# MaxLayar/Ray-Tracing-Extended

Measured on AMD Instinct MI355X. Metric: Mrays/s, higher is better.
Workload: dtype f32; 1 GPU; configs[2]: Chess pieces x17 (100,440 triangles, BVH4), 1920x1080, 64 rays/pixel/frame (1024 spp = 16 frames), 8 bounces, PCG, FLAT_CHUNKS semantics; decomposition=single GPU, rays_per_frame=243378252, triangles=100440, chunks=7448, spheres=0

## Files before the change

### ray-tracing-extended_amd/csrc/rt_api.hip

```cpp
#include <hip/hip_runtime.h>

#include <algorithm>
#include <chrono>
#include <cfloat>
#include <cmath>
#include <condition_variable>
#include <deque>
#include <mutex>
#include <cstdarg>
#include <cstdio>
#include <cstring>
#include <ctime>
#include <string>
#include <thread>
#include <vector>

#include "rt_kernels.hpp"
#include "rt_stream.hpp"
namespace rtk {
const void* stream_kernel(bool counting, bool philox, bool compact, bool triangles);
const void* cam_stream_kernel(bool philox, bool compact, bool triangles);
}
#include "rt_geom.hpp"
#include "rt_bvh_gpu.hpp"
// ... 38 lines not shown
    int row0 = 0, nrows = -1;
    int band_first = 0, band_stride = 0;

    std::vector<rt_sphere>   h_spheres;
    std::vector<rt_triangle> h_tris;
    std::vector<rt_meshinfo> h_mesh;
    bool scene_dirty = true;
    size_t n_tris = 0, n_chunks = 0, n_spheres = 0;
    float sphere_mag = 0.f;
    bool geom_local = false, xf_dirty = false;
    uint64_t frames_traced = 0, frames_at_world_build = ~0ull;
    std::vector<rt_triangle>       h_local_tris;
    std::vector<rt_local_chunk>    h_lchunks;
    std::vector<rt_mesh_transform> h_xf;
    std::vector<float>             mesh_radius;
    int n_meshes = 0;
    DevBuf<float> d_local_tris;
    DevBuf<uint32_t> d_tri_mesh, d_tri_chunk, d_tri_rank, d_order;
    DevBuf<rtg::MeshXf> d_xf;
    hipEvent_t evg0 = nullptr, evg1 = nullptr;
    hipEvent_t ev_switch = nullptr;

    DevBuf<float4> d_sph_geom, d_sph_mat, d_nodes, d_nodes_h, d_tri_geo, d_tri_nrm, d_chunk_mat, d_chunk_box;
    DevBuf<float>  d_raw_tris;
    DevBuf<uint32_t> d_raw_range;
    DevBuf<float4> d_frame, d_accum;
    DevBuf<uint32_t> d_display;
    DevBuf<float4> d_batch;
    DevBuf<uint32_t> d_tile_order, d_tile_cost, d_tile_hist;
    bool lpt_active = true;
    bool tile_order_valid = false, tile_order_stale = false; int tile_order_n = 0;
    size_t target_pixels = 0;
    int target_w = 0, target_h = 0, target_row0 = 0, target_rows = 0, target_row_stride = 8;
    unsigned int* d_tile_counter = nullptr;
    unsigned long long* d_counters = nullptr;

    rtbvh::Bvh bvh;
    size_t n_nodes = 0;
    rtgb::Workspace bvh_ws;
    float area_at_build = 0.f;
    float area_after_refit = 0.f;
    int opt_device_bvh = -1;
    int opt_bvh_radius = -16;
    int opt_peer_copies = 0;
    int opt_bvh_treelet_ratio = 8, opt_bvh_treelet_isolate = 1, opt_bvh_treelet_first = 1;
    int opt_bvh_treelets = 6;
    int opt_bvh_top = 0;
    int opt_rebuild_percent = 200;
    int n_cu = 0;
    int opt_kernel = -1;
    int auto_choice = -1; double auto_ms[2] = { -1.0, -1.0 };
    unsigned variants_launched = 0;
    int opt_shade_threshold = 48;
    int opt_tile_sync = 1;
    int opt_fetch_guide = 4;
    int opt_fetch_guide_philox = 1;
    int opt_tiles_per_fetch = 16;
    int opt_compact_nodes = 1;
    int opt_stream_tile = 4;
    int opt_node_min = 10;
    int opt_blocks_per_cu = 0;
    int opt_full_sort = 0;
    int opt_tile_lpt = 1;
    int opt_frame_batch = 0;
    int opt_tile_w_log2 = 3;
    int opt_bvh_reinsert = 0;
    int opt_bvh_bins = 32, opt_bvh_cost_exp = 100;
    int opt_max_leaf = 2;
    int opt_bvh_collapse = 0;
    int opt_bvh_node_cost = 130;
    int opt_stream_stack = 0;
    int opt_lds_stack = 0;
    DevBuf<uint32_t> d_gstack;
    DevBuf<uint4> d_primary; DevBuf<float4> d_focus; DevBuf<unsigned int> d_primary_counts;
    std::string primary_key;
    unsigned long long scene_version = 0;
    int opt_primary_lists = 1;
    DevBuf<float> d_park;
    std::vector<rtk::CamRecord> h_cams; DevBuf<rtk::CamRecord> d_cams;
    DevBuf<float4> d_q_rays, d_q_hits; DevBuf<uint8_t> d_q_occ;
    DevBuf<unsigned int> d_q_bound;
    DevBuf<float4> d_aov[RT_AOV_COUNT];
    size_t aov_pixels = 0;
    int aov_w = 0, aov_h = 0, aov_row0 = 0, aov_rows = 0, aov_row_stride = 8;
    rt_aov_info aov{};
    rt_stats stats{};

    std::thread q_thread; bool q_started = false;
    std::mutex q_mu; std::condition_variable q_cv, q_idle;
    struct QItem { int frame; rt_params p; };
    std::deque<QItem> q_frames; bool q_busy = false, q_stop = false;
    rt_params q_tail{};
    int q_rc = 0; std::string q_err;
    int opt_queue_depth = 64;
    int opt_queue_linger_us = 200;
};

namespace {

int fail(rt_ctx* ctx, int code, const char* fmt, ...)
{
    char buf[512];
    va_list ap; va_start(ap, fmt); vsnprintf(buf, sizeof buf, fmt, ap); va_end(ap);
    if (ctx) ctx->err = buf; else g_create_error = buf;
    return code;
}
// ... 477 lines not shown
        F.tile_w_log2 = c->opt_tile_w_log2;
        const int tw = 1 << F.tile_w_log2, th = 64 >> F.tile_w_log2;
        F.tiles_x = (c->target_w + tw - 1) / tw; F.tiles_y = (c->target_rows + th - 1) / th;
    }
    const bool philox = P.philox = c->params.rngMode == RT_RNG_PHILOX && c->params.numRaysPerPixel >= 1;
    if (philox && var == Variant::Flat) return fail(c, -2, "the flat validation kernel implements the PCG stream only");
    if (philox) kernel = 1;
    if (philox && (c->target_w > 65535 || c->target_rows > 65535)) return fail(c, -7, "the Philox mode addresses at most 65535 x 65535 pixels per context");
    if (philox && (c->params.numRaysPerPixel > 65000 || c->params.maxBounceCount > 32000))
        return fail(c, -7, "the Philox mode takes at most 65000 rays per pixel per frame and 32000 bounces (sample and bounce share one signed 32-bit register)");
    const bool stream = P.stream = kernel == 1 && var != Variant::Flat && c->params.numRaysPerPixel >= 1
                                   && c->target_w <= 65535 && c->target_rows <= 65535
                                   && c->params.numRaysPerPixel <= 65000 && c->params.maxBounceCount <= 32000;
    const bool tile_kernel = P.tile_kernel = !stream && var != Variant::Flat;
    F.stack_cap = tile_kernel ? tile_stack_cap(c)
                              : std::max(1, c->bvh.maxStack) + (stream ? 3 : 0);
    const bool seven_waves = stream && !philox && var == Variant::Fast && c->opt_compact_nodes != 0 && c->n_nodes > 0;
    const int stream_stack = c->opt_stream_stack > 0 ? c->opt_stream_stack : (seven_waves ? (RT_STREAM_WAVES >= 7 ? 21 : 24) : 30);
    const bool stream_spill = stream && F.stack_cap > stream_stack;
    if (stream_spill) F.stack_cap = stream_stack;
    F.full_sort = c->opt_full_sort;
    bool fixed_origin = camera_origin_is_fixed(c->params);
    if (cams) for (int f = 0; f < n_frames; ++f) fixed_origin = fixed_origin && camera_origin_is_fixed(cams[f]);
    F.fixed_origin = fixed_origin ? 1 : 0;
    F.out_frame = c->d_frame.p; F.accum = c->d_accum.p;
    F.tile_counter = c->d_tile_counter; F.counters = c->d_counters;

    const size_t lds = P.lds = var == Variant::Flat ? 0
                                       : (size_t)F.stack_cap * 64 * sizeof(uint32_t) * rtk::kWavesPerBlock
                                         + (stream ? (size_t)rtk::kGroupMax * sizeof(uint2) * rtk::kWavesPerBlock : 0);
    if (lds > 160 * 1024) return fail(c, -7, "BVH needs a %d-entry traversal stack: exceeds the 160 KiB LDS", F.stack_cap);
    const bool counting = var == Variant::Counting;
    const bool compact = c->opt_compact_nodes != 0;
    P.cam_table = cams != nullptr;
    const void* fn = P.fn = var == Variant::Flat ? (const void*)rtk::k_trace<false, true>
                   : stream ? (cams ? rtk::cam_stream_kernel(philox, compact, c->n_nodes > 0)
                                    : rtk::stream_kernel(counting, philox, compact, c->n_nodes > 0))
                   : c->n_nodes == 0
                            ? dispatch3(counting, false, false, [](auto C, auto, auto) { return (const void*)rtk::k_trace<decltype(C)::value, false, false, 6>; })
                            : dispatch3(counting, false, compact, [](auto C, auto, auto H) { return (const void*)rtk::k_trace<decltype(C)::value, false, decltype(H)::value>; });
    if (lds > 64 * 1024) RT_HIP(c, hipFuncSetAttribute(fn, hipFuncAttributeMaxDynamicSharedMemorySize, (int)lds));
    int per_cu = 0;
    RT_HIP(c, hipOccupancyMaxActiveBlocksPerMultiprocessor(&per_cu, fn, rtk::kBlock, lds));
    if (per_cu < 1) return fail(c, -7, "kernel does not fit a CU (LDS %zu B)", lds);
    P.ntiles = F.tiles_x * F.tiles_y;
    P.sample_lanes_log2 = !philox ? 0 : c->params.numRaysPerPixel >= 16 ? 4 : c->params.numRaysPerPixel >= 4 ? 2 : 0;
    const bool stream_sync = P.stream_sync = stream && (c->opt_tile_sync || philox);
    if (cams && !stream_sync) return fail(c, -7, "per-frame cameras: no k_cam_stream launch for this target");
    const size_t frames_in_queue = ((stream_sync && c->opt_frame_batch != 1) ? (size_t)std::max(1, std::min(n_frames, 64)) : 1) << P.sample_lanes_log2;
    const int want = (int)std::min<size_t>(((size_t)P.ntiles * frames_in_queue + rtk::kWavesPerBlock - 1) / rtk::kWavesPerBlock, (size_t)1 << 20);
    if (c->opt_blocks_per_cu > 0) per_cu = std::min(per_cu, c->opt_blocks_per_cu);
    const int grid = P.grid = std::max(1, std::min(want, per_cu * c->n_cu));
    A.shade_threshold = std::max(1, std::min(64, c->opt_shade_threshold));
    A.total_pixels = (unsigned int)P.ntiles * 64u;
    A.tile_sync = stream_sync ? 1 : 0;
    A.sample_lanes_log2 = P.sample_lanes_log2;
    A.tiles_per_fetch = std::max(1, std::min(rtk::kGroupMax, c->opt_tiles_per_fetch));
    A.guide_div = 1;
    A.node_min = std::max(1, std::min(64, c->opt_node_min));
    const unsigned int gstack_stride = (unsigned int)grid * rtk::kBlock;
    if (philox) {
        RT_HIP(c, c->d_park.ensure((size_t)grid * rtk::kWavesPerBlock * (size_t)A.tiles_per_fetch * 192));
        F.park = c->d_park.p;
    }
    if (stream_spill) {
        RT_HIP(c, c->d_gstack.ensure((size_t)(c->bvh.maxStack + 3 - F.stack_cap) * gstack_stride));
        F.gstack = c->d_gstack.p; F.gstack_stride = gstack_stride;
    }
    if (tile_kernel && c->bvh.maxStack > F.stack_cap) {
        RT_HIP(c, c->d_gstack.ensure((size_t)(c->bvh.maxStack - F.stack_cap) * gstack_stride));
        F.gstack = c->d_gstack.p; F.gstack_stride = gstack_stride;
    }
    if ((tile_kernel || stream_sync) && n_frames > 1 && c->opt_frame_batch != 1) {
        const size_t budget = (size_t)4 << 30;
        const size_t per_frame = c->target_pixels * sizeof(float4);
        int batch = (int)std::min<size_t>((size_t)n_frames, std::max<size_t>(1, budget / per_frame));
        if (c->opt_frame_batch > 1) batch = std::min(batch, c->opt_frame_batch);
        P.batch = batch = std::min(batch, 256);
        if (batch > 1) RT_HIP(c, c->d_batch.ensure((size_t)batch * c->target_pixels));
    }
    return 0;
}

int plan_tile_order(rt_ctx* c, LaunchPlan& P)
{
    const int ntiles = P.ntiles;
    const bool lpt = (P.tile_kernel || P.stream_sync) && c->opt_tile_lpt && ntiles > 1;
    c->lpt_active = lpt;
    if (!lpt) return 0;
    if (c->tile_order_n != ntiles) { c->tile_order_valid = false; c->tile_order_n = ntiles; }
    RT_HIP(c, c->d_tile_cost.ensure(ntiles)); RT_HIP(c, c->d_tile_order.ensure(ntiles));
    if (!c->tile_order_valid || c->tile_order_stale) {
        P.record_costs = true;
        RT_HIP(c, hipMemsetAsync(c->d_tile_cost.p, 0, (size_t)ntiles * sizeof(uint32_t), c->stream));
    }
    P.F.tile_order = c->tile_order_valid ? c->d_tile_order.p : nullptr;
    P.F.tile_cost = P.record_costs ? c->d_tile_cost.p : nullptr;
    return 0;
}

int ensure_primary_lists(rt_ctx* c, LaunchPlan& P)
{
    const bool eligible = P.stream && !P.cam_table && c->opt_primary_lists && c->n_nodes > 0 && P.F.fixed_origin && c->target_pixels > 0
                          && c->bvh.maxStack <= 160;
    if (!eligible) return 0;
    std::string key((const char*)&c->params, sizeof c->params);
// ... 606 lines not shown
        }
    }
    for (int t = 0; t < n_tris; ++t) if (!seen[t]) return fail(c, -5, "triangle %d belongs to no chunk", t);
    for (float& r : radius) r *= 1.7320508f;
    c->h_local_tris.assign(tris, tris + n_tris); c->h_lchunks.assign(chunks, chunks + n_chunks);
    c->mesh_radius = radius; c->n_meshes = n_meshes;
    c->geom_local = true; c->scene_dirty = true;
    return 0;
}

int rt_set_mesh_transforms(rt_ctx* c, const rt_mesh_transform* xf, int n_meshes)
{
    if (!c) return -1;
    RT_SETTLE(c);
    if (n_meshes < 0 || (n_meshes > 0 && !xf)) return fail(c, -2, "bad transform upload");
    if (c->geom_local && n_meshes != c->n_meshes) return fail(c, -2, "%d transforms for %d meshes", n_meshes, c->n_meshes);
    c->h_xf.assign(xf, xf + n_meshes);
    c->xf_dirty = true;
    return 0;
}

int rt_read_world_geometry(rt_ctx* c, rt_triangle* tris_out, int n_tris, rt_meshinfo* mi_out, int n_chunks)
{
    if (!c) return -1;
    RT_SETTLE(c);
    if (!c->geom_local) return fail(c, -2, "no local meshes uploaded");
    if (!c->have_params) return fail(c, -2, "rt_set_params has not been called");
    if (n_tris != (int)c->h_local_tris.size() || n_chunks != (int)c->h_lchunks.size()) return fail(c, -2, "size mismatch");
    RT_HIP(c, hipSetDevice(c->device));
    { int r = prepare_scene(c); if (r) return r; }
    if (n_tris) RT_HIP(c, hipMemcpy(tris_out, c->d_raw_tris.p, (size_t)n_tris * sizeof(rt_triangle), hipMemcpyDeviceToHost));
    std::vector<float4> box(2 * (size_t)n_chunks);
    if (n_chunks) RT_HIP(c, hipMemcpy(box.data(), c->d_chunk_box.p, box.size() * sizeof(float4), hipMemcpyDeviceToHost));
    for (int m = 0; m < n_chunks; ++m) {
        const rt_local_chunk& ch = c->h_lchunks[m];
        rt_meshinfo& mi = mi_out[m];
        mi.firstTriangleIndex = ch.firstTriangleIndex; mi.numTriangles = ch.numTriangles; mi.material = ch.material;
        mi.boundsMin[0] = box[2 * m].x; mi.boundsMin[1] = box[2 * m].y; mi.boundsMin[2] = box[2 * m].z;
        mi.boundsMax[0] = box[2 * m + 1].x; mi.boundsMax[1] = box[2 * m + 1].y; mi.boundsMax[2] = box[2 * m + 1].z;
    }
    return 0;
}

int rt_set_option(rt_ctx* c, const char* name, int value)
{
    if (!c) return -1;
    RT_SETTLE(c);
    if (!name) return fail(c, -2, "null option name");
    if (!std::strcmp(name, "kernel")) {
        if (value < -1 || value > 1) return fail(c, -2, "kernel must be -1 (auto), 0 (k_trace) or 1 (k_stream)");
        c->opt_kernel = value;
    }
    else if (!std::strcmp(name, "shade_threshold")) { if (value < 1 || value > 64) return fail(c, -2, "shade_threshold must be in [1,64]"); c->opt_shade_threshold = value; }
    else if (!std::strcmp(name, "stream_stack")) { if (value != 0 && (value < 4 || value > 128)) return fail(c, -2, "stream_stack must be 0 (automatic) or in [4,128]"); c->opt_stream_stack = value; }
    else if (!std::strcmp(name, "lds_stack")) { if (value < 0 || value > 64) return fail(c, -2, "lds_stack must be in [0,64]"); c->opt_lds_stack = value; }
    else if (!std::strcmp(name, "bvh_bins")) { if (value < 2 || value > 128) return fail(c, -2, "bvh_bins must be in [2,128]"); if (value != c->opt_bvh_bins) c->scene_dirty = true; c->opt_bvh_bins = value; }
    else if (!std::strcmp(name, "bvh_reinsert")) { if (value < 0 || value > 16) return fail(c, -2, "bvh_reinsert must be in [0,16]"); if (value != c->opt_bvh_reinsert) c->scene_dirty = true; c->opt_bvh_reinsert = value; }
    else if (!std::strcmp(name, "bvh_cost_exp")) { if (value < 10 || value > 300) return fail(c, -2, "bvh_cost_exp must be in [10,300] (percent)"); if (value != c->opt_bvh_cost_exp) c->scene_dirty = true; c->opt_bvh_cost_exp = value; }
    else if (!std::strcmp(name, "max_leaf")) { if (value < 1 || value > rtbvh::kMaxLeaf) return fail(c, -2, "max_leaf must be in [1,4]"); if (value != c->opt_max_leaf) c->scene_dirty = true; c->opt_max_leaf = value; }
    else if (!std::strcmp(name, "bvh_collapse")) { if (value < 0 || value > 2) return fail(c, -2, "bvh_collapse must be 0 (greedy), 1 (cost-driven, leaves formed by the collapse) or 2 (cost-driven over the split search's leaves)"); if (value != c->opt_bvh_collapse) c->scene_dirty = true; c->opt_bvh_collapse = value; }
    else if (!std::strcmp(name, "bvh_node_cost")) { if (value < 1 || value > 10000) return fail(c, -2, "bvh_node_cost must be in [1,10000] (percent of a triangle test)"); if (value != c->opt_bvh_node_cost) c->scene_dirty = true; c->opt_bvh_node_cost = value; }
    else if (!std::strcmp(name, "tile_w_log2")) { if (value < 0 || value > 6) return fail(c, -2, "tile_w_log2 must be in [0,6]"); c->opt_tile_w_log2 = value; }
    else if (!std::strcmp(name, "tile_lpt")) { c->opt_tile_lpt = value ? 1 : 0; c->tile_order_valid = false; }
    else if (!std::strcmp(name, "frame_batch")) { if (value < 0 || value > 1024) return fail(c, -2, "frame_batch must be in [0,1024]"); c->opt_frame_batch = value; }
    else if (!std::strcmp(name, "fetch_guide")) { if (value < 1 || value > 64) return fail(c, -2, "fetch_guide must be in [1,64]"); c->opt_fetch_guide = value; }
    else if (!std::strcmp(name, "fetch_guide_philox")) { if (value < 1 || value > 64) return fail(c, -2, "fetch_guide_philox must be in [1,64]"); c->opt_fetch_guide_philox = value; }
    else if (!std::strcmp(name, "tiles_per_fetch")) { if (value < 1 || value > 64) return fail(c, -2, "tiles_per_fetch must be in [1,64]"); c->opt_tiles_per_fetch = value; }
    else if (!std::strcmp(name, "node_min")) { if (value < 1 || value > 64) return fail(c, -2, "node_min must be in [1,64]"); c->opt_node_min = value; }
    else if (!std::strcmp(name, "tile_sync")) c->opt_tile_sync = value ? 1 : 0;
    else if (!std::strcmp(name, "compact_nodes")) c->opt_compact_nodes = value ? 1 : 0;
    else if (!std::strcmp(name, "device_bvh")) { if (value < -1 || value > 1) return fail(c, -2, "device_bvh must be -1 (automatic), 0 or 1"); if (value != c->opt_device_bvh) c->scene_dirty = true; c->opt_device_bvh = value; }
    else if (!std::strcmp(name, "bvh_radius")) { if (value == 0 || value < -rtgb::kMaxRadius || value > rtgb::kMaxRadius) return fail(c, -2, "bvh_radius must be in [1,64] (negative: the same radius in every round)"); if (value != c->opt_bvh_radius) c->scene_dirty = true; c->opt_bvh_radius = value; }
    else if (!std::strcmp(name, "peer_copies")) { if (value != 0 && value != 1) return fail(c, -2, "peer_copies must be 0 or 1"); c->opt_peer_copies = value; }
    else if (!std::strcmp(name, "bvh_treelet_ratio")) { if (value < 2 || value > 64) return fail(c, -2, "bvh_treelet_ratio must be in [2,64]"); if (value != c->opt_bvh_treelet_ratio) c->scene_dirty = true; c->opt_bvh_treelet_ratio = value; }
    else if (!std::strcmp(name, "bvh_treelet_isolate")) { if (value < 0 || value > 1) return fail(c, -2, "bvh_treelet_isolate must be 0 or 1"); if (value != c->opt_bvh_treelet_isolate) c->scene_dirty = true; c->opt_bvh_treelet_isolate = value; }
    else if (!std::strcmp(name, "bvh_treelet_first")) { if (value < 1 || value > 4096) return fail(c, -2, "bvh_treelet_first must be in [1,4096]"); if (value != c->opt_bvh_treelet_first) c->scene_dirty = true; c->opt_bvh_treelet_first = value; }
    else if (!std::strcmp(name, "bvh_treelets")) { if (value < 0 || value > 16) return fail(c, -2, "bvh_treelets must be in [0,16] (passes)"); if (value != c->opt_bvh_treelets) c->scene_dirty = true; c->opt_bvh_treelets = value; }
    else if (!std::strcmp(name, "bvh_top")) { if (value < 0 || value > (1 << 20)) return fail(c, -2, "bvh_top must be in [0,1048576] (0 = the device's clustering builds the whole tree)"); if (value != c->opt_bvh_top) c->scene_dirty = true; c->opt_bvh_top = value; }
    else if (!std::strcmp(name, "rebuild_percent")) { if (value < 0 || value > 100000) return fail(c, -2, "rebuild_percent must be in [0,100000] (0 = never rebuild)"); c->opt_rebuild_percent = value; }
    else if (!std::strcmp(name, "stream_tile")) { if (value != 0 && value != 2 && value != 4) return fail(c, -2, "stream_tile must be 0 (8x8 pixels x 1 frame), 2 (4x4 x 4 frames) or 4 (2x2 x 16 frames)"); c->opt_stream_tile = value; }
    else if (!std::strcmp(name, "full_sort")) c->opt_full_sort = value ? 1 : 0;
    else if (!std::strcmp(name, "primary_lists")) { if (value != 0 && value != 1) return fail(c, -2, "primary_lists must be 0 or 1"); c->opt_primary_lists = value; }
    else if (!std::strcmp(name, "queue_depth")) { if (value < 1 || value > 256) return fail(c, -2, "queue_depth must be in [1,256]"); c->opt_queue_depth = value; }
    else if (!std::strcmp(name, "queue_linger_us")) { if (value < 0 || value > 1000000) return fail(c, -2, "queue_linger_us must be in [0,1000000]"); c->opt_queue_linger_us = value; }
    else if (!std::strcmp(name, "blocks_per_cu")) { if (value < 0) return fail(c, -2, "blocks_per_cu must be >= 0"); c->opt_blocks_per_cu = value; }
    else return fail(c, -2, "unknown option '%s'", name);
    return 0;
}

int rt_set_rows(rt_ctx* c, int row0, int nrows)
{
    if (!c) return -1;
    RT_SETTLE(c);
    if (row0 < 0 || nrows < 0) return fail(c, -2, "bad row strip (%d,%d)", row0, nrows);
    c->row0 = row0; c->nrows = nrows; c->band_stride = 0;
    return 0;
}

int rt_set_bands(rt_ctx* c, int first_band, int band_stride)
{
    if (!c) return -1;
    RT_SETTLE(c);
    if (first_band < 0 || band_stride < 1 || first_band >= band_stride) return fail(c, -2, "bad band pattern (%d,%d)", first_band, band_stride);
    c->band_first = first_band; c->band_stride = band_stride;
    return 0;
}
// ... 581 lines not shown
```

### ray-tracing-extended_amd/csrc/rt_stream.hpp

```cpp
#pragma once
#include "rt_kernels.hpp"

namespace rtk {

struct StreamArgs {
    int shade_threshold;
    unsigned int total_pixels;
    int node_min;
    int tiles_per_fetch;
    int guide_div;
    int tile_sync;
    int n16, n4, n1;
    int sample_lanes_log2;
};

enum : uint32_t { kModeTrav = 0, kModeShade = 1, kModeDead = 2, kModeWait = 3, kModeTravStrict = 0xFFFFFFFFu };
__device__ __forceinline__ bool is_trav(uint32_t mode) { return (int)mode <= 0; }
constexpr uint32_t kNoPixel = 0xFFFFFFFFu;

struct StreamKernArgs { DeviceScene S; FrameArgs F; StreamArgs A; };
static_assert(alignof(StreamArgs) <= 8, "kernarg layout = struct layout");
static_assert(offsetof(StreamKernArgs, F) == ((sizeof(DeviceScene) + 7) & ~size_t(7))
              && offsetof(StreamKernArgs, A) == ((offsetof(StreamKernArgs, F) + sizeof(FrameArgs) + 7) & ~size_t(7)), "kernarg layout = struct layout");

struct CamRecord {
    float4 view;
    float4 m0, m1, m2;
    float4 pos;
};
struct StreamCamKernArgs { DeviceScene S; FrameArgs F; StreamArgs A; const CamRecord* cams; };
static_assert(offsetof(StreamCamKernArgs, A) == offsetof(StreamKernArgs, A)
              && offsetof(StreamCamKernArgs, cams) == ((offsetof(StreamCamKernArgs, A) + sizeof(StreamArgs) + 7) & ~size_t(7)), "kernarg layout = struct layout");

#ifndef RT_STREAM_WAVES
#define RT_STREAM_WAVES 7
#endif
#ifndef RT_STREAM_WAVES_PHILOX
#define RT_STREAM_WAVES_PHILOX 5
#endif
constexpr int stream_waves(bool count, bool philox, bool h, bool tri) { return count ? 3 : !tri ? 6 : philox ? RT_STREAM_WAVES_PHILOX : !h ? 5 : RT_STREAM_WAVES; }


template <bool COUNT, bool PHILOX = false, bool H = false, bool TRI = true>
__global__ __launch_bounds__(kBlock) __attribute__((amdgpu_waves_per_eu(stream_waves(COUNT, PHILOX, H, TRI), stream_waves(COUNT, PHILOX, H, TRI)))) void k_stream(DeviceScene S, FrameArgs F, StreamArgs A)
{
    constexpr bool CAMS = false;
#include "rt_stream_body.hpp"
}

template <bool PHILOX, bool H, bool TRI>
__global__ __launch_bounds__(kBlock) __attribute__((amdgpu_waves_per_eu(stream_waves(false, PHILOX, H, TRI), stream_waves(false, PHILOX, H, TRI)))) void k_cam_stream(DeviceScene S, FrameArgs F, StreamArgs A, const CamRecord* cams)
{
    constexpr bool COUNT = false, CAMS = true;
    (void)cams;
#include "rt_stream_body.hpp"
}

}
```

### ray-tracing-extended_amd/csrc/rt_stream_body.hpp

```cpp
    extern __shared__ uint32_t lds_stack[];
    RT_MARK("begin prologue");
    const int lane = threadIdx.x & 63, wave = threadIdx.x >> 6;
    uint32_t* stk = lds_stack + (size_t)wave * F.stack_cap * 64 + lane;
    const int cap = F.stack_cap;
    uint32_t* const gstk = F.gstack ? F.gstack + (blockIdx.x * kBlock + threadIdx.x) : nullptr;
    using lds_u32 = __attribute__((address_space(3))) uint32_t;
    const uint32_t stk0 = (uint32_t)(uintptr_t)(lds_u32*)stk;
    uint32_t top = stk0;
    auto slot = [](uint32_t a) -> lds_u32& { return *reinterpret_cast<lds_u32*>((uintptr_t)a); };
    const uint32_t capb = (uint32_t)cap << 8;
    uint32_t ub = 0u;
    auto pop = [&]() -> uint32_t {
        top -= 256u;
        if (gstk == nullptr || ub <= capb) return slot(top);
        RT_RARE_PATH();
        const uint32_t depth = top - stk0;
        uint32_t v = slot(stk0 + min(depth, capb - 256u));
        asm volatile("" : "+v"(v));
        if (depth >= capb) { RT_RARE_PATH(); v = gstk[(size_t)((depth - capb) >> 8) * F.gstack_stride]; }
        return v;
    };
    typedef uint32_t u32x2 __attribute__((ext_vector_type(2)));
    using lds_u2 = __attribute__((address_space(3))) u32x2;
    lds_u2* const item_tab = reinterpret_cast<lds_u2*>((uintptr_t)__builtin_amdgcn_readfirstlane(
// ... 10 lines not shown
    uint32_t rng = 0u;
    int sample = 0;
    v3 total = rtm::mk(0.f, 0.f, 0.f), light = total, rayColour = total, o = total, d = total;
    RaySlabT<H> slab = make_slab<H>(rtm::mk(0.f, 0.f, 0.f), rtm::mk(1.f, 1.f, 1.f));
    uint32_t cur = kNone;
    Hit best; best.t = INF; best.id = kNone; best.u = 0.f; best.v = 0.f;
    bool live = false;
    unsigned long long wave_t0 = 0;
    unsigned int group_base = 0, group_len = 0;
    unsigned int next_unit = 0;
    unsigned int kidx = 0;

    auto decode = [](const FrameArgs& F, const StreamArgs& A, unsigned int item, unsigned int& tile, unsigned int& sub, unsigned int& frame0) -> int {
        const unsigned int ntiles_ = (unsigned)(F.tiles_x * F.tiles_y);
        if constexpr (PHILOX) {
            const int sgl = A.sample_lanes_log2;
            const unsigned int per_frame = ntiles_ << sgl;
            const unsigned int g = item / per_frame, r = item - g * per_frame;
            tile = r >> sgl; sub = r & ((1u << sgl) - 1u); frame0 = g;
            return sgl;
        }
        const unsigned int items1_ = (unsigned)A.n1 * ntiles_, items4_ = (unsigned)A.n4 * (ntiles_ << 2);
        int fgl = 0; unsigned int fbase = (unsigned)A.n16 * 16u + (unsigned)A.n4 * 4u;
        if (item >= items1_) { item -= items1_; fgl = 2; fbase = (unsigned)A.n16 * 16u; if (item >= items4_) { item -= items4_; fgl = 4; fbase = 0u; } }
        const unsigned int per_group = ntiles_ << fgl;
        const unsigned int g = item / per_group, r = item - g * per_group;
        tile = r >> fgl; sub = r & ((1u << fgl) - 1u); frame0 = fbase + (g << fgl);
        return fgl;
    };
    auto pixel_index = [&](const FrameArgs& F) -> uint32_t {
        const int ly = (int)(pxy >> 16);
        return (uint32_t)(F.row0 + (ly >> 3) * F.row_stride + (ly & 7)) * (uint32_t)F.p.width + (pxy & 0xFFFFu);
    };
    auto start_pixel = [&](const FrameArgs& F, const StreamArgs& A, unsigned int id) -> bool {
        const rt_params& p = F.p;
        const uint32_t W = (uint32_t)p.width;
        const unsigned int nframes_ = (unsigned)(A.n16 * 16 + A.n4 * 4 + A.n1);
        const u32x2 e = item_tab[id >> 6];
        const unsigned int pos = id & 63u;
        const int fgl = (int)(e.y >> 28);
        const unsigned int frame0 = e.y & 0x0FFFFFFFu;
        const int pxl = 6 - fgl, swl = pxl >> 1;
        const unsigned int pix = pos & ((1u << pxl) - 1u);
        const unsigned int fi = PHILOX ? frame0 : frame0 + (pos >> pxl);
        const int x = (int)((e.x & 0xFFFFu) + (pix & ((1u << swl) - 1u)));
        const int yy = (int)((e.x >> 16) + (pix >> swl));
        if (!(x < p.width && yy < F.nrows && fi < nframes_)) return false;
        pxy = (uint32_t)x | ((uint32_t)yy << 16); kidx = id | (fi << 16);
        const uint32_t pixelIndex = (uint32_t)(F.row0 + (yy >> 3) * F.row_stride + (yy & 7)) * W + (uint32_t)x;
        if constexpr (PHILOX) sample = (int)(pos >> pxl);
        else { rng = pixelIndex + (uint32_t)(F.frame + (int)fi) * 719393u; sample = 0; }
        total = rtm::mk(0.f, 0.f, 0.f);
        live = false;
        return true;
    };
    auto take_units = [&](const FrameArgs& F, const StreamArgs& A, bool want) -> bool {
        bool got = false;
        const unsigned int total_units = group_len << 6;
        for (;;) {
            const unsigned long long need = ballot_(want);
            if (need == 0ull || next_unit >= total_units) break;
            if (want) {
                const unsigned int id = next_unit + __builtin_amdgcn_mbcnt_hi((uint32_t)(need >> 32), __builtin_amdgcn_mbcnt_lo((uint32_t)need, 0u));
                if (id < total_units && start_pixel(F, A, id)) { want = false; got = true; }
            }
            next_unit = __builtin_amdgcn_readfirstlane(min(total_units, next_unit + (unsigned int)__popcll(need)));
        }
        return got;
    };

    RT_MARK("end prologue");
    for (;;) {
        const int nTrav = __popcll(ballot_(is_trav(mode))), nShade = __popcll(ballot_(mode == kModeShade));
        if (nTrav + nShade == 0) {
            if (!A.tile_sync) break;
            RT_REGION_BEGIN(fetch);
            const StreamKernArgs& KA = fresh_kernargs<StreamKernArgs>();
            const FrameArgs& F = KA.F; const StreamArgs& A = KA.A;
            const unsigned int ntiles_ = (unsigned)(F.tiles_x * F.tiles_y);
            const unsigned int nitems_ = PHILOX ? (unsigned)A.n1 * (ntiles_ << A.sample_lanes_log2)
                                                : (unsigned)A.n1 * ntiles_ + (unsigned)A.n4 * (ntiles_ << 2) + (unsigned)A.n16 * (ntiles_ << 4);
            if constexpr (PHILOX) {
                const int pxl = 6 - A.sample_lanes_log2, swl = pxl >> 1;
                const uint32_t W = (uint32_t)F.p.width;
                const float nf = (float)F.p.numRaysPerPixel;
                asm volatile("s_waitcnt vmcnt(0)" ::: "memory");
                for (unsigned int k = 0; k < group_len; ++k) {
                    const u32x2 e = item_tab[k];
                    const unsigned int fi = e.y & 0x0FFFFFFFu;
                    const unsigned int pix = (unsigned)lane & ((1u << pxl) - 1u);
                    const int x = (int)((e.x & 0xFFFFu) + (pix & ((1u << swl) - 1u)));
                    const int yy = (int)((e.x >> 16) + (pix >> swl));
                    const bool present = x < F.p.width && yy < F.nrows;
                    float tx = 0.f, ty = 0.f, tz = 0.f;
                    if (present) {
                        const float* q = park_slot(F, A, k) + lane;
                        tx = __hip_atomic_load(q, __ATOMIC_RELAXED, __HIP_MEMORY_SCOPE_AGENT);
                        ty = __hip_atomic_load(q + 64, __ATOMIC_RELAXED, __HIP_MEMORY_SCOPE_AGENT);
                        tz = __hip_atomic_load(q + 128, __ATOMIC_RELAXED, __HIP_MEMORY_SCOPE_AGENT);
                    }
                    for (int off = 1 << pxl; off < 64; off <<= 1) {
                        tx = tx + __shfl_xor(tx, off, 64); ty = ty + __shfl_xor(ty, off, 64); tz = tz + __shfl_xor(tz, off, 64);
                    }
                    if (present && ((unsigned)lane >> pxl) == 0u) {
                        const float cx = tx / nf, cy = ty / nf, cz = tz / nf;
                        const size_t pi = (size_t)yy * W + (uint32_t)x;
                        F.out_frame[(size_t)fi * F.frame_stride + pi] = make_float4(cx, cy, cz, 1.0f);
                        if (F.frames_in_launch <= 1) {
                            const float weight = 1.0f / (float)(F.frame + 1);
                            const float omw = 1.0f - weight;
                            const float4 prev = F.accum[pi];
                            float4 acc;
                            acc.x = rtm::saturate(prev.x * omw + cx * weight);
                            acc.y = rtm::saturate(prev.y * omw + cy * weight);
                            acc.z = rtm::saturate(prev.z * omw + cz * weight);
                            acc.w = rtm::saturate(prev.w * omw + 1.0f * weight);
                            F.accum[pi] = acc;
                        }
                    }
                }
            }
            uint32_t slot = (uint32_t)lane;
            asm volatile("" : "+v"(slot));
            if (F.tile_cost && group_len != 0 && slot < group_len) {
                const uint32_t share = (uint32_t)(((__builtin_readcyclecounter() - wave_t0) >> 6) / group_len);
                const u32x2 e = item_tab[slot];
                atomicAdd(&F.tile_cost[((e.x >> 16) >> 3) * (unsigned)F.tiles_x + ((e.x & 0xFFFFu) >> 3)], share);
            }
            unsigned int base = 0, K = 1;
            if (lane == 0) {
                const unsigned int handed = __hip_atomic_load(F.tile_counter, __ATOMIC_RELAXED, __HIP_MEMORY_SCOPE_AGENT) >> 6;
                const unsigned int rem = nitems_ > handed ? nitems_ - handed : 0u;
                K = min((unsigned)A.tiles_per_fetch, max(1u, rem / (unsigned)A.guide_div));
                base = atomicAdd(F.tile_counter, 64u * K);
            }
            base = __builtin_amdgcn_readfirstlane(base);
            K = __builtin_amdgcn_readfirstlane(K);
            group_base = base >> 6;
            if (group_base >= nitems_) break;
            group_len = min(K, nitems_ - group_base);
            wave_t0 = __builtin_readcyclecounter();
            if (slot < group_len) {
                unsigned int tile, sub, frame0;
                const int fgl = decode(F, A, group_base + slot, tile, sub, frame0);
                const int swl = (6 - fgl) >> 1;
                if (F.tile_order) tile = F.tile_order[tile];
                const unsigned int x0 = (tile % (unsigned)F.tiles_x) * 8u + ((sub & ((1u << (3 - swl)) - 1u)) << swl);
                const unsigned int y0 = (tile / (unsigned)F.tiles_x) * 8u + ((sub >> (3 - swl)) << swl);
                item_tab[slot] = u32x2{ x0 | (y0 << 16), frame0 | ((unsigned)fgl << 28) };
            }
            next_unit = 0;
            if (take_units(F, A, true)) { fresh = true; mode = kModeShade; }
            RT_REGION_END(fetch);
            continue;
        }

        const int thr = min(A.shade_threshold, (A.shade_threshold * (nTrav + nShade) + 63) >> 6);
        if (nShade >= thr || nTrav == 0) {
            __builtin_amdgcn_s_setprio(0);
            RT_REGION_BEGIN(shade);
            const StreamKernArgs& KA = fresh_kernargs<StreamKernArgs>();
            const DeviceScene& S = KA.S; const FrameArgs& F = KA.F; const StreamArgs& A = KA.A;
            const rt_params& p = F.p;
            const float* M = p.camLocalToWorld;
            const uint32_t W = (uint32_t)p.width;
            bool need_ray = false;
            bool want = false;
            bool retrace = false;
            if (mode == kModeShade) {
                need_ray = fresh;
                fresh = false;
                bool path_done = false;
                if constexpr (TRI) {
                    if (live && best.id != kNone && (best.id & kTriBit) && p.intersectMode == RT_INTERSECT_FLAT_CHUNKS) {
                        RT_REGION_BEGIN(verify);
                        const uint32_t chunk = __float_as_uint(S.tri_nrm[(size_t)(best.id & ~kTriBit) * 3].w);
                        const float4 bmn = S.chunk_box[(size_t)chunk * 2], bmx = S.chunk_box[(size_t)chunk * 2 + 1];
                        if (!ray_bounding_box(o, slab.inv, rtm::mk(bmn.x, bmn.y, bmn.z), rtm::mk(bmx.x, bmx.y, bmx.z))) { retrace = true; live = false; }
                        RT_REGION_END(verify);
                    }
                }
                if (live) {
                    if (best.id != kNone) {
                        RT_REGION_BEGIN(hit);
                        phase_tick<COUNT>(cnt, 2);
                        if (COUNT) cnt.hits++;
                        const v3 hitPoint = o + d * best.t;
                        v3 normal; const float4* mat;
                        if (best.id & kTriBit) {
                            const uint32_t ti = best.id & ~kTriBit;
                            const float4* tn = S.tri_nrm + (size_t)ti * 3;
                            const float4 n0 = tn[0], n1 = tn[1], n2 = tn[2];
                            const float w = 1.0f - best.u - best.v;
                            normal = rtm::normalize((rtm::mk(n0.x, n0.y, n0.z) * w + rtm::mk(n1.x, n1.y, n1.z) * best.u)
                                                    + rtm::mk(n2.x, n2.y, n2.z) * best.v);
                            mat = S.chunk_mat + (size_t)__float_as_uint(n0.w) * 4;
                        } else {
                            RT_REGION_BEGIN(hit_sphere);
                            const float4 s = S.sph_geom[best.id];
                            normal = rtm::normalize(hitPoint - rtm::mk(s.x, s.y, s.z));
                            mat = S.sph_mat + (size_t)best.id * 4;
                            RT_REGION_END(hit_sphere);
                        }
                        const float4 mcol = mat[0], memi = mat[1], mprm = mat[3];
                        const int flag = (int)__float_as_uint(mprm.w);
                        v3 colour = rtm::mk(mcol.x, mcol.y, mcol.z);
                        bool skip = false;
                        if (flag == 1) {
                            RT_REGION_BEGIN(hit_checker);
                            float cx = mod2(__builtin_floorf(hitPoint.x)), cz = mod2(__builtin_floorf(hitPoint.z));
                            if (!(cx == cz)) colour = rtm::mk(memi.x, memi.y, memi.z);
                            RT_REGION_END(hit_checker);
                        } else if (flag == 2 && (sample >> 16) == 0) {
                            o = hitPoint + d * 0.001f;
                            skip = true;
                        }
                        if (!skip) {
                            RT_REGION_BEGIN(hit_scatter);
                            auto scatter = [&](auto& R) {
                                const bool isSpecular = mprm.z >= rtm::random_value(R);
                                const float specF = isSpecular ? 1.0f : 0.0f;
                                o = hitPoint;
// ... 16 lines not shown
                            RT_REGION_END(hit_scatter);
                        }
                        sample += 0x10000;
                        if ((sample >> 16) > p.maxBounceCount) path_done = true;
                        RT_REGION_END(hit);
                    } else {
                        RT_REGION_BEGIN(env);
#if !defined(RT_DIAG_IDLE) && !defined(RT_DIAG_PRIMARY) && !defined(RT_DIAG_TOP) && !defined(RT_DIAG_STACK)
                        phase_tick<COUNT>(cnt, 3);
#endif
                        light = light + environment_light(p, d) * rayColour;
                        path_done = true;
                        RT_REGION_END(env);
                    }
                    if (path_done) {
                        total = total + light;
                        sample = (sample & 0xFFFF) + (PHILOX ? 1 << A.sample_lanes_log2 : 1);
                        if (PHILOX && sample >= p.numRaysPerPixel) {
                            float* q = park_slot(F, A, (kidx & 0xFFFFu) >> 6) + (kidx & 63u);
                            q[0] = total.x; q[64] = total.y; q[128] = total.z;
                            pxy = kNoPixel; want = true;
                        } else if (sample >= p.numRaysPerPixel) {
                            RT_REGION_BEGIN(pixel_done);
                            const float n = (float)p.numRaysPerPixel;
                            const float cx = total.x / n, cy = total.y / n, cz = total.z / n;
                            const size_t pi = (size_t)(pxy >> 16) * W + (pxy & 0xFFFFu);
                            float one = 1.0f;
                            asm volatile("" : "+v"(one));
                            F.out_frame[(size_t)(kidx >> 16) * F.frame_stride + pi] = make_float4(cx, cy, cz, one);
                            if (F.frames_in_launch <= 1) {
                                const float weight = 1.0f / (float)(F.frame + 1);
                                const float omw = 1.0f - weight;
                                const float4 prev = F.accum[pi];
                                float4 acc;
                                acc.x = rtm::saturate(prev.x * omw + cx * weight);
                                acc.y = rtm::saturate(prev.y * omw + cy * weight);
                                acc.z = rtm::saturate(prev.z * omw + cz * weight);
                                acc.w = rtm::saturate(prev.w * omw + 1.0f * weight);
                                F.accum[pi] = acc;
                            }
                            pxy = kNoPixel; want = A.tile_sync != 0;
                            RT_REGION_END(pixel_done);
                        } else need_ray = true;
                    }
                    live = false;
                }
            }
            if (ballot_(want) != 0ull) {
                RT_REGION_BEGIN(take);
                const bool got = take_units(F, A, want);
                if (want) { if (got) need_ray = true; else mode = kModeWait; }
                RT_REGION_END(take);
            }
            if (mode == kModeShade) {
                while (!PHILOX && !A.tile_sync) {
                    const unsigned long long need = ballot_(pxy == kNoPixel && mode != kModeDead);
                    if (need == 0) break;
                    RT_REGION_BEGIN(refill);
                    if (pxy == kNoPixel && mode != kModeDead) {
                        unsigned int base = 0;
                        const int first = __builtin_ctzll(need);
                        if (lane == first) base = atomicAdd(F.tile_counter, (unsigned int)__popcll(need));
                        base = __shfl(base, first, 64);
                        const unsigned int idx = base + (unsigned int)__popcll(need & ((1ull << lane) - 1ull));
                        if (idx >= A.total_pixels) mode = kModeDead;
                        else {
                            const unsigned int tile = idx >> 6, within = idx & 63u;
                            const int x = (int)(tile % (unsigned)F.tiles_x) * 8 + (int)(within & 7u);
                            const int yy = (int)(tile / (unsigned)F.tiles_x) * 8 + (int)(within >> 3);
                            if (x < p.width && yy < F.nrows) {
                                pxy = (uint32_t)x | ((uint32_t)yy << 16);
                                const int y = F.row0 + (yy >> 3) * F.row_stride + (yy & 7);
                                rng = ((uint32_t)y * W + (uint32_t)x) + (uint32_t)F.frame * 719393u;
                                total = rtm::mk(0.f, 0.f, 0.f);
                                sample = 0;
                                need_ray = true;
                            }
                        }
                    }
                    RT_REGION_END(refill);
                }
                if (mode == kModeShade) {
                    if (need_ray) {
                        RT_REGION_BEGIN(camera);
#if !defined(RT_DIAG_IDLE) && !defined(RT_DIAG_PRIMARY) && !defined(RT_DIAG_TOP) && !defined(RT_DIAG_STACK)
                        phase_tick<COUNT>(cnt, 4);
#endif
                        Camera cam;
                        cam.W = (float)W;
                        if constexpr (CAMS) {
                        auto rec = [&]() { return fresh_kernargs<StreamCamKernArgs>().cams + (kidx >> 16); };
                        const int px = (int)(pxy & 0xFFFFu), ly = (int)(pxy >> 16);
                        const int y = F.row0 + (ly >> 3) * F.row_stride + (ly & 7);
                        const float4 vw = rec()->view;
                        const float uvx = ((float)px + 0.5f) / cam.W, uvy = ((float)y + 0.5f) / (float)(uint32_t)p.height;
                        const float lx = (uvx - 0.5f) * vw.x, lyv = (uvy - 0.5f) * vw.y, lz = 1.0f * vw.z;
                        const float4 r0 = rec()->m0;
                        const float fx = ((r0.x * lx + r0.y * lyv) + r0.z * lz) + r0.w * 1.0f;
                        const float4 r1 = rec()->m1;
                        const float fy = ((r1.x * lx + r1.y * lyv) + r1.z * lz) + r1.w * 1.0f;
                        const float4 r2 = rec()->m2;
                        cam.focusPoint = rtm::mk(fx, fy, ((r2.x * lx + r2.y * lyv) + r2.z * lz) + r2.w * 1.0f);
                        const CamRecord* rc = rec();
                        cam.right = rtm::mk(rc->m0.x, rc->m1.x, rc->m2.x);
                        cam.up    = rtm::mk(rc->m0.y, rc->m1.y, rc->m2.y);
                        const float4 pv = rc->pos;
                        cam.pos   = rtm::mk(pv.x, pv.y, pv.z);
// ... 155 lines not shown
                            else { cur = kNone; mode = kModeShade; }
                            RT_REGION_END(node_pop);
                        }
                        RT_REGION_END(node);
                    }
                    RT_REGION_END(nodeloop);
                }
                if (is_trav(mode) && (int)cur < 0) {
                    RT_REGION_BEGIN(leaf);
                    uint32_t ti = (cur & 0x7FFFFFFFu) >> 2;
                    const uint32_t last = ti + (cur & 3u);
                    if (cur != kNone)
                    for (; ti <= last; ++ti) {
                        RT_REGION_BEGIN(tri);
                        float4 g0, g1, g2;
                        load_tri(S.tri_geo, ti, g0, g1, g2);
                        float dst, u, v;
                        if (COUNT) cnt.tris++;
                        phase_tick<COUNT>(cnt, 1);
#ifdef RT_DIAG_PRIMARY
                        if (COUNT && (sample >> 16) == 0) { cnt.phase_lanes[4]++; if ((unsigned)__builtin_ctzll(ballot_(true)) == (unsigned)lane) cnt.phase_execs[4]++; }
#endif
                        const bool hit = ray_triangle(o, d, rtm::mk(g0.x, g0.y, g0.z), rtm::mk(g0.w, g1.x, g1.y),
                                                      rtm::mk(g1.z, g1.w, g2.x), rtm::mk(g2.y, g2.z, g2.w), dst, u, v);
                        if (hit && dst <= best.t) {
                            RT_REGION_BEGIN(tri_accept);
                            bool take = dst < best.t;
                            if (!take && (best.id & kTriBit) && best.id != kNone) {
                                RT_REGION_BEGIN(tri_tie);
                                uint32_t oc = __float_as_uint(S.tri_nrm[(size_t)ti * 3 + 1].w);
                                uint32_t ob = __float_as_uint(S.tri_nrm[(size_t)(best.id & ~kTriBit) * 3 + 1].w);
                                take = oc < ob;
                                RT_REGION_END(tri_tie);
                            }
                            if (take && mode == kModeTravStrict) {
                                RT_RARE_PATH();
                                RT_REGION_BEGIN(tri_chunk);
                                uint32_t chunk = __float_as_uint(S.tri_nrm[(size_t)ti * 3].w);
                                float4 bmn = S.chunk_box[(size_t)chunk * 2], bmx = S.chunk_box[(size_t)chunk * 2 + 1];
                                take = ray_bounding_box(o, slab.inv, rtm::mk(bmn.x, bmn.y, bmn.z), rtm::mk(bmx.x, bmx.y, bmx.z));
                                RT_REGION_END(tri_chunk);
                            }
                            if (take) { best.t = dst; best.id = kTriBit | ti; best.u = u; best.v = v; }
                            RT_REGION_END(tri_accept);
                        }
                        RT_REGION_END(tri);
                    }
                    if (top != stk0) cur = pop();
                    else { cur = kNone; mode = kModeShade; }
                    RT_REGION_END(leaf);
                }
                RT_REGION_END(burstiter);
                if (ballot_(is_trav(mode)) == 0) break;
                if ((int)__popcll(ballot_(mode == kModeShade)) >= thr) break;
            }
            RT_REGION_END(burst);
            }
        }
    }
    RT_MARK("begin epilogue");
    {
        unsigned long long v[kNumCounters] = { cnt.rays, cnt.sph, cnt.nodes, cnt.tris, cnt.hits };
        for (int k = 0; k < 5; ++k) { v[5 + k] = cnt.phase_lanes[k]; v[10 + k] = cnt.phase_execs[k]; }
        for (int k = 0; k < kNumRegions; ++k) v[15 + k] = cnt.region[k];
        for (int k = 0; k < (COUNT ? kNumCounters : 1); ++k) {
            unsigned long long s = v[k];
#ifdef RT_DIAG_STACK
            if (k == 8) {
                for (int off = 32; off > 0; off >>= 1) s = max(s, (unsigned long long)__shfl_down(s, off, 64));
                if (lane == 0) atomicMax(&fresh_kernargs<StreamKernArgs>().F.counters[k], s);
                continue;
            }
#endif
            for (int off = 32; off > 0; off >>= 1) s += __shfl_down(s, off, 64);
            if (lane == 0) atomicAdd(&fresh_kernargs<StreamKernArgs>().F.counters[k], s);
        }
    }
    RT_MARK("end epilogue");
```

Before: 21220 Mrays/s.

## Split wavefront shading into separate hit and miss batches with own thresholds

Lanes waiting to shade are now counted separately as hits and misses. The shade phase can run for just the hit group or just the miss group once that group reaches its own threshold (defaults 40 and 20, scaled by occupancy), and traversal bursts can end early on the same condition. The aim is less divergence inside the shading code, since hit shading and miss shading take different paths, and shorter waits for a full batch. In exchange, shade phases become more frequent and smaller, there are extra ballots every iteration, and traversal is interrupted more often.

```diff
diff --git a/ray-tracing-extended_amd/csrc/rt_api.hip b/ray-tracing-extended_amd/csrc/rt_api.hip
--- a/ray-tracing-extended_amd/csrc/rt_api.hip
+++ b/ray-tracing-extended_amd/csrc/rt_api.hip
@@ -114,6 +114,7 @@
     int auto_choice = -1; double auto_ms[2] = { -1.0, -1.0 };
     unsigned variants_launched = 0;
     int opt_shade_threshold = 48;
+    int opt_shade_hit_min = 40, opt_shade_miss_min = 20;
     int opt_tile_sync = 1;
     int opt_fetch_guide = 4;
     int opt_fetch_guide_philox = 1;
@@ -697,6 +698,8 @@
     if (c->opt_blocks_per_cu > 0) per_cu = std::min(per_cu, c->opt_blocks_per_cu);
     const int grid = P.grid = std::max(1, std::min(want, per_cu * c->n_cu));
     A.shade_threshold = std::max(1, std::min(64, c->opt_shade_threshold));
+    A.shade_hit_min = std::max(0, std::min(64, c->opt_shade_hit_min));
+    A.shade_miss_min = std::max(0, std::min(64, c->opt_shade_miss_min));
     A.total_pixels = (unsigned int)P.ntiles * 64u;
     A.tile_sync = stream_sync ? 1 : 0;
     A.sample_lanes_log2 = P.sample_lanes_log2;
@@ -1409,6 +1412,8 @@
         c->opt_kernel = value;
     }
     else if (!std::strcmp(name, "shade_threshold")) { if (value < 1 || value > 64) return fail(c, -2, "shade_threshold must be in [1,64]"); c->opt_shade_threshold = value; }
+    else if (!std::strcmp(name, "shade_hit_min")) { if (value < 0 || value > 64) return fail(c, -2, "shade_hit_min must be in [0,64]"); c->opt_shade_hit_min = value; }
+    else if (!std::strcmp(name, "shade_miss_min")) { if (value < 0 || value > 64) return fail(c, -2, "shade_miss_min must be in [0,64]"); c->opt_shade_miss_min = value; }
     else if (!std::strcmp(name, "stream_stack")) { if (value != 0 && (value < 4 || value > 128)) return fail(c, -2, "stream_stack must be 0 (automatic) or in [4,128]"); c->opt_stream_stack = value; }
     else if (!std::strcmp(name, "lds_stack")) { if (value < 0 || value > 64) return fail(c, -2, "lds_stack must be in [0,64]"); c->opt_lds_stack = value; }
     else if (!std::strcmp(name, "bvh_bins")) { if (value < 2 || value > 128) return fail(c, -2, "bvh_bins must be in [2,128]"); if (value != c->opt_bvh_bins) c->scene_dirty = true; c->opt_bvh_bins = value; }
diff --git a/ray-tracing-extended_amd/csrc/rt_stream.hpp b/ray-tracing-extended_amd/csrc/rt_stream.hpp
--- a/ray-tracing-extended_amd/csrc/rt_stream.hpp
+++ b/ray-tracing-extended_amd/csrc/rt_stream.hpp
@@ -12,6 +12,8 @@
     int tile_sync;
     int n16, n4, n1;
     int sample_lanes_log2;
+    int shade_hit_min;
+    int shade_miss_min;
 };
 
 enum : uint32_t { kModeTrav = 0, kModeShade = 1, kModeDead = 2, kModeWait = 3, kModeTravStrict = 0xFFFFFFFFu };
diff --git a/ray-tracing-extended_amd/csrc/rt_stream_body.hpp b/ray-tracing-extended_amd/csrc/rt_stream_body.hpp
--- a/ray-tracing-extended_amd/csrc/rt_stream_body.hpp
+++ b/ray-tracing-extended_amd/csrc/rt_stream_body.hpp
@@ -86,6 +86,7 @@
         else { rng = pixelIndex + (uint32_t)(F.frame + (int)fi) * 719393u; sample = 0; }
         total = rtm::mk(0.f, 0.f, 0.f);
         live = false;
+        best.id = kNone;
         return true;
     };
     auto take_units = [&](const FrameArgs& F, const StreamArgs& A, bool want) -> bool {
@@ -105,7 +106,8 @@
 
     RT_MARK("end prologue");
     for (;;) {
-        const int nTrav = __popcll(ballot_(is_trav(mode))), nShade = __popcll(ballot_(mode == kModeShade));
+        const unsigned long long mShade = ballot_(mode == kModeShade);
+        const int nTrav = __popcll(ballot_(is_trav(mode))), nShade = __popcll(mShade);
         if (nTrav + nShade == 0) {
             if (!A.tile_sync) break;
             RT_REGION_BEGIN(fetch);
@@ -190,7 +192,13 @@
         }
 
         const int thr = min(A.shade_threshold, (A.shade_threshold * (nTrav + nShade) + 63) >> 6);
-        if (nShade >= thr || nTrav == 0) {
+        const unsigned long long mHit = mShade & ballot_(best.id != kNone);
+        const int nHit = __popcll(mHit), nMiss = nShade - nHit;
+        const int hit_min = A.shade_hit_min > 0 ? min(A.shade_hit_min, (A.shade_hit_min * (nTrav + nShade) + 63) >> 6) : 65;
+        const int miss_min = A.shade_miss_min > 0 ? min(A.shade_miss_min, (A.shade_miss_min * (nTrav + nShade) + 63) >> 6) : 65;
+        const bool serve_all = nShade >= thr || nTrav == 0;
+        const bool serve_hit = serve_all || nHit >= hit_min, serve_miss = serve_all || nMiss >= miss_min;
+        if (serve_hit || serve_miss) {
             __builtin_amdgcn_s_setprio(0);
             RT_REGION_BEGIN(shade);
             const StreamKernArgs& KA = fresh_kernargs<StreamKernArgs>();
@@ -201,7 +209,8 @@
             bool need_ray = false;
             bool want = false;
             bool retrace = false;
-            if (mode == kModeShade) {
+            const bool served = mode == kModeShade && (best.id != kNone ? serve_hit : serve_miss);
+            if (served) {
                 need_ray = fresh;
                 fresh = false;
                 bool path_done = false;
@@ -324,7 +333,7 @@
                 if (want) { if (got) need_ray = true; else mode = kModeWait; }
                 RT_REGION_END(take);
             }
-            if (mode == kModeShade) {
+            if (served && mode == kModeShade) {
                 while (!PHILOX && !A.tile_sync) {
                     const unsigned long long need = ballot_(pxy == kNoPixel && mode != kModeDead);
                     if (need == 0) break;
@@ -586,7 +595,14 @@
                 }
                 RT_REGION_END(burstiter);
                 if (ballot_(is_trav(mode)) == 0) break;
-                if ((int)__popcll(ballot_(mode == kModeShade)) >= thr) break;
+                const unsigned long long done = ballot_(mode == kModeShade);
+                const int nDone = __popcll(done);
+                if (nDone >= thr) break;
+                if (min(hit_min, miss_min) <= 64) {
+                    const int nDoneHit = __popcll(done & ballot_(best.id != kNone));
+                    if (nDoneHit >= hit_min) break;
+                    if (nDone - nDoneHit >= miss_min) break;
+                }
             }
             RT_REGION_END(burst);
             }
```

Result: no change. 21220 Mrays/s, median of 2 (-0.0%).
